# KrArunT/whisper-rust-ort

Hardware: AMD Instinct MI355X
Metric: rtfx: audio seconds transcribed per wall second (whisper-base, 30 s clips, greedy 128 new tokens) (higher is better)
Workload: dtype bf16

## Files before the change

whisper-rust-ort_amd/binding.py:

```python
from __future__ import annotations

import ctypes as C
import os
from dataclasses import dataclass
from typing import List, Optional, Sequence, Tuple

import numpy as np

HERE = os.path.dirname(os.path.abspath(__file__))
LIB_PATH = os.path.join(HERE, "libwhisper_hip.so")

WH_PREC_F32, WH_PREC_BF16, WH_PREC_FP8, WH_PREC_F16X3 = 0, 1, 2, 3
PRECISIONS = {"f32": WH_PREC_F32, "bf16": WH_PREC_BF16, "fp8": WH_PREC_FP8, "f16x3": WH_PREC_F16X3}
WH_N_FRAMES, WH_CLIP_SAMPLES = 3000, 480000
WH_PCM_S16, WH_PCM_U8, WH_PCM_F32 = 0, 1, 2
WH_MAX_CHANNELS = 64
PCM_FORMATS = {np.dtype(np.int16): WH_PCM_S16, np.dtype(np.uint8): WH_PCM_U8, np.dtype(np.float32): WH_PCM_F32}
KG_NAMES = ("mel", "enc_gemm", "enc_attn", "dec_cross_attn", "dec_gemm", "dec_other")

STATUS = {0: "WH_OK", 1: "WH_ERR_EMPTY_AUDIO", 2: "WH_ERR_BAD_SHAPE", 3: "WH_ERR_STATE", 4: "WH_ERR_ARG",
          5: "WH_ERR_NOMEM", 6: "WH_ERR_HIP", 7: "WH_ERR_IO", 8: "WH_ERR_UNSUPPORTED"}

EXPORTS = ("wh_model_load", "wh_model_create", "wh_model_free", "wh_model_get_dims", "wh_model_precision",
           "wh_model_export_tensor", "wh_ctx_create", "wh_ctx_create_ex", "wh_ctx_free", "wh_ctx_cross_mode", "wh_ctx_placement", "wh_last_error", "wh_get_timings",
# ... 325 lines not shown
            rc = self.lib.wh_ctx_create_ex(model.h, C.byref(o), C.byref(h))
        if rc:
            raise WhisperHipError(rc, (self.lib.wh_last_error(None) or b"").decode())
        self.h = h

    def _check(self, rc: int):
        if rc:
            raise WhisperHipError(rc, (self.lib.wh_last_error(self.h) or b"").decode())

    @property
    def cross_mode(self) -> int:
        return int(self.lib.wh_ctx_cross_mode(self.h))

    @property
    def placement(self) -> dict:
        a, b = C.c_float(0), C.c_float(0)
        n = int(self.lib.wh_ctx_placement(self.h, C.byref(a), C.byref(b)))
        return {"workspaces_timed": n, "first_us_per_launch": float(a.value), "kept_us_per_launch": float(b.value)}

    def debug_set_step_split(self, rows: int):
        self._check(self.lib.wh_debug_set_step_split(self.h, C.c_int(rows)))

    @property
    def step_split(self) -> int:
        return int(self.lib.wh_debug_get_step_split(self.h))

    def debug_set_step_free(self, on: bool):
        self._check(self.lib.wh_debug_set_step_free(self.h, C.c_int(1 if on else 0)))

    @property
    def step_free(self) -> int:
        return int(self.lib.wh_debug_get_step_free(self.h))

    def set_timestamp_rules(self, tb: int, no_timestamps: int = -1, max_initial_index: int = 50):
        r = WhTimestampRules(C.sizeof(WhTimestampRules), tb, no_timestamps, max_initial_index)
        self._check(self.lib.wh_ctx_set_timestamp_rules(self.h, C.byref(r)))

    def clear_timestamp_rules(self):
        self._check(self.lib.wh_ctx_set_timestamp_rules(self.h, None))

    def set_logprobs(self, no_speech: int = -1, sot_index: int = 0):
        o = WhLogprobOpts(C.sizeof(WhLogprobOpts), no_speech, sot_index)
        self._check(self.lib.wh_ctx_set_logprobs(self.h, C.byref(o)))

    def clear_logprobs(self):
        self._check(self.lib.wh_ctx_set_logprobs(self.h, None))

    def logprobs(self) -> Tuple[List[np.ndarray], Optional[np.ndarray]]:
        n = C.c_size_t(0)
        self._check(self.lib.wh_get_logprobs(self.h, None, 0, None, 0, C.byref(n)))
        k = int(n.value)
        lens = list(self._gen_lens)
        assert len(lens) == k, (len(lens), k)
        cap = max(1, max(lens, default=0))
        lp = np.zeros((max(1, k), cap), np.float32)
        ns = np.zeros(max(1, k), np.float32)
        rc = self.lib.wh_get_logprobs(self.h, _f32(lp), cap, _f32(ns), k, C.byref(n))
        if rc == 3:
            ns = None
            rc = self.lib.wh_get_logprobs(self.h, _f32(lp), cap, None, k, C.byref(n))
        self._check(rc)
        return [lp[i, : lens[i]].copy() for i in range(k)], (ns[:k] if ns is not None else None)

    def set_language_detection(self, ids: Sequence[int], sot_index: int = 0):
        a = np.ascontiguousarray(list(ids), np.int64)
        o = WhLanguageOpts(C.sizeof(WhLanguageOpts), _i64(a) if a.size else None, a.size, sot_index)
# ... 614 lines not shown
```

whisper-rust-ort_amd/build.py:

```python
from __future__ import annotations

import os
import subprocess
import sys
from concurrent.futures import ThreadPoolExecutor

HERE = os.path.dirname(os.path.abspath(__file__))
CSRC = os.path.join(HERE, "csrc")
OUT = os.path.join(HERE, "libwhisper_hip.so")
SOURCES = ["wh_lm_head.hip", "wh_dec_gemm.hip", "wh_mel.hip", "wh_ingest.hip", "wh_gemm.hip", "wh_gemm8.hip", "wh_gemm8x.hip", "wh_gemm8_mx.hip", "wh_mlp.hip", "wh_attn.hip", "wh_dec_attn.hip", "wh_dec_tile.hip", "wh_cross_es.hip", "wh_cross_es8.hip", "wh_cross_es3.hip", "wh_fp8.hip", "wh_align.hip", "wh_beam.hip", "wh_sample.hip", "wh_score.hip", "wh_model.cpp", "wh_ctx.cpp", "wh_options.cpp", "wh_encode_host.cpp", "wh_decode_host.cpp", "wh_score_host.cpp", "wh_api.cpp"]
HEADERS = ["wh_common.h", "wh_es_common.h", "wh_dec_epilogue.h", "wh_kernels.h", "wh_lm_tile.h", "wh_internal.h", "wh_host_shared.h", "wh_step.h", "wh_ingest_desc.h", "wh_json.h", "../../include/whisper_hip.h"]
FLAGS = ["--offload-arch=gfx950", "-O3", "-fPIC", "-std=c++17", "-pthread", "-Wall", "-Wno-unused-function", "-Wno-unused-value", "-Wno-unused-result",
         "-mllvm", "-amdgpu-mfma-vgpr-form=1", "-x", "hip"]


EXTRA_FLAGS = {"wh_attn.hip": ["-fno-honor-nans"], "wh_cross_es.hip": ["-fno-honor-nans"], "wh_cross_es8.hip": ["-fno-honor-nans"], "wh_cross_es3.hip": ["-fno-honor-nans"]}


def _stale(target: str, deps) -> bool:
    if not os.path.exists(target):
        return True
    t = os.path.getmtime(target)
    return any(os.path.getmtime(d) > t for d in deps)


def build(verbose: bool = False, force: bool = False) -> str:
    hipcc = os.environ.get("HIPCC", "/opt/rocm/bin/hipcc")
    objdir = os.path.join(HERE, "build")
    os.makedirs(objdir, exist_ok=True)
    hdrs = [os.path.join(CSRC, h) for h in HEADERS]

    def compile_one(src: str) -> str:
        s = os.path.join(CSRC, src)
        o = os.path.join(objdir, src + ".o")
        if force or _stale(o, [s] + hdrs):
            cmd = [hipcc] + FLAGS + EXTRA_FLAGS.get(src, []) + ["-c", s, "-o", o]
            if verbose:
                print(" ".join(cmd), flush=True)
            subprocess.check_call(cmd)
        return o

    with ThreadPoolExecutor(max_workers=min(6, os.cpu_count() or 1)) as ex:
        objs = list(ex.map(compile_one, SOURCES))
    if force or _stale(OUT, objs):
        cmd = [hipcc, "--offload-arch=gfx950", "-shared", "-fPIC", "-pthread", "-o", OUT] + objs
        if verbose:
            print(" ".join(cmd), flush=True)
        subprocess.check_call(cmd)
    build_host(verbose, force)
    build_tools(verbose, force)
    return OUT


TOOLS = os.path.join(HERE, "..", "tools")


def build_tools(verbose: bool = False, force: bool = False) -> None:
    hipcc = os.environ.get("HIPCC", "/opt/rocm/bin/hipcc")
    for name, kernel_src in (("mx_mfma_check", "wh_gemm8_mx.hip"), ("mx_gemm_check", "wh_gemm8_mx.hip"), ("mlp_check", "wh_mlp.hip"), ("es16_check", "wh_cross_es.hip"), ("es8_check", "wh_cross_es8.hip"), ("es3_check", "wh_cross_es3.hip"), ("align_check", "wh_align.hip")):
        src, exe = os.path.join(TOOLS, name + ".hip"), os.path.join(TOOLS, name)
        deps = [src, os.path.join(CSRC, kernel_src), os.path.join(CSRC, "wh_common.h"), os.path.join(CSRC, "wh_es_common.h"), os.path.join(CSRC, "wh_dec_epilogue.h"), os.path.join(CSRC, "wh_kernels.h")]
        if force or _stale(exe, deps):
            cmd = [hipcc, "--offload-arch=gfx950", "-O3", "-std=c++17", "-mllvm", "-amdgpu-mfma-vgpr-form=1"] + EXTRA_FLAGS.get(kernel_src, []) + ["-w", "-I", CSRC, src, "-o", exe]
            if verbose:
                print(" ".join(cmd), flush=True)
            subprocess.check_call(cmd)
    for name in ("dec_gemm_check", "enc_check", "dec_attn_check", "lm_check"):
        src, exe = os.path.join(TOOLS, name + ".cpp"), os.path.join(TOOLS, name)
        if force or _stale(exe, [src, OUT, os.path.join(CSRC, "wh_kernels.h")]):
            cmd = [hipcc, "--offload-arch=gfx950", "-O2", "-std=c++17", "-w", src, "-o", exe, "-L" + HERE, "-lwhisper_hip", "-Wl,-rpath,$ORIGIN/../whisper-rust-ort_amd"]
            if verbose:
                print(" ".join(cmd), flush=True)
            subprocess.check_call(cmd)


HOST = os.path.join(HERE, "host")
HOST_SO = os.path.join(HERE, "libwh_host.so")
CLI = os.path.join(HERE, "whisper_bench")


def build_host(verbose: bool = False, force: bool = False) -> None:
    gxx = os.environ.get("CXX", "g++")
    import ctypes
    try:
        ctypes.CDLL("libz.so.1")
    except OSError as e:
        raise RuntimeError(f"libz.so.1 is missing: whisper_bench --temperature and libwh_host.so's compression_ratio need zlib ({e})") from e
    hdr =[os.path.join(HOST, "wh_host.h"), os.path.join(HOST, "wh_unicode_lower.h"), os.path.join(CSRC, "wh_json.h"), os.path.join(HERE, "..", "include", "whisper_hip.h")]
    src = os.path.join(HOST, "wh_host_capi.cpp")
    if force or _stale(HOST_SO, [src] + hdr):
        cmd = [gxx, "-O2", "-std=c++17", "-fPIC", "-shared", "-Wall", "-o", HOST_SO, src, "-ldl"]
        if verbose:
            print(" ".join(cmd), flush=True)
        subprocess.check_call(cmd)
    src = os.path.join(HOST, "whisper_bench.cpp")
    if force or _stale(CLI, [src, OUT] + hdr):
        cmd = [gxx, "-O2", "-std=c++17", "-Wall", "-pthread", "-D__HIP_PLATFORM_AMD__", "-I/opt/rocm/include", "-o", CLI, src, "-L" + HERE, "-lwhisper_hip",
               "-Wl,-rpath,$ORIGIN", "-Wl,-rpath,/opt/rocm/lib", "-L/opt/rocm/lib", "-lamdhip64", "-ldl"]
        if verbose:
            print(" ".join(cmd), flush=True)
# ... 6 lines not shown
```

whisper-rust-ort_amd/csrc/wh_ctx.cpp:

```cpp
#include "wh_host_shared.h"

using namespace wh;

namespace wh {

int fail(wh_ctx* c, int code, const char* fmt, ...) {
    char buf[1024];
    va_list ap;
    va_start(ap, fmt);
    vsnprintf(buf, sizeof buf, fmt, ap);
    va_end(ap);
    if (c) c->err = buf;
    wh_set_error("%s", buf);
    return code;
}

void prof_reset(wh_ctx* c) {
    for (int g = 0; g < WH_KG_COUNT; g++) { c->prof_used[g] = 0; c->prof_ms[g] = 0; c->prof_launches[g] = 0; }
}
void prof_collect(wh_ctx* c) {
    if (!c->prof) return;
    for (int g = 0; g < WH_KG_COUNT; g++) {
        double ms = 0;
        for (size_t i = 0; i < c->prof_used[g]; i++) {
// ... 148 lines not shown
    c->sm.timing = getenv("WH_SAMPLE_TIMING") != nullptr;
    c->sc.timing = getenv("WH_SCORE_TIMING") != nullptr;
    const wh_dims& D = m->dims;
    const size_t B = max_batch, d = D.d_model, S = D.n_audio_ctx, F = D.ffn, C = D.n_mels, esz = m->esz;
    const size_t Ld = D.dec_layers, H = D.n_heads, TC = D.n_text_ctx;
    c->ldv = (int)align_up(S, 64);
    c->tok_ld = D.n_text_ctx + 1;
    c->mpad = (int)align_up(B, B > 16 ? 64 : 16);
    c->cross_splits = (int)std::min<size_t>(32, std::max<size_t>(1, 256 / B));
    if (m->prec == WH_PREC_BF16 && d > 512 && d % 256 == 0)
        c->cross_splits = (int)std::min<size_t>(32, std::max<size_t>(1, 512 / (B * (d / 256))));
    const size_t n_tiles = (D.vocab + 15) / 16;
    Carver cv;
    const size_t o_pcm = cv.take(B * WH_CLIP_SAMPLES * 4), o_raw = cv.take(B * C * RAW_LD * 4);
    const size_t o_melstage = cv.take(C * WH_N_FRAMES * 4);
    const size_t o_melT = cv.take((B * TOK_ROWS * C + 256) * esz), o_h1 = cv.take((B * H1_ROWS * d + 256) * esz);
    const size_t o_x = cv.take(B * S * d * 4), o_xn = cv.take(B * S * d * esz), o_qk = cv.take(B * S * 2 * d * esz);
    c->enc_fold = m->prec == WH_PREC_BF16 && max_batch > WH_SMALL_CTX_CLIPS && d >= 256 && (d % 64) == 0 && (F % 64) == 0 && S >= 256 && (S % 4) == 0 &&
                  m->cross_kv_wf != nullptr && wh_gemm8_enabled() && getenv("WH_NO_ENC_FOLD") == nullptr;
    c->enc_mlp = c->enc_fold && d == 512 && F >= 128 && (F % 128) == 0 && !(getenv("WH_ENC_MLP") && atoi(getenv("WH_ENC_MLP")) == 0);
    const size_t o_vT = cv.take(B * d * c->ldv * esz), o_att = cv.take(B * S * d * esz), o_h = c->enc_mlp ? 0 : cv.take(B * S * F * esz);
    const size_t o_enc = cv.take(B * S * d * esz), o_encf = cv.take(B * S * d * 4);
    c->cross_es = m->cross_es && max_batch >= 256;
    if (opts->flags & WH_CTX_CROSS_ES_ON) c->cross_es = m->cross_es;
    if (opts->flags & WH_CTX_CROSS_ES_OFF) c->cross_es = false;
    if (const char* e = getenv("WH_CROSS_ES")) c->cross_es = m->cross_es && atoi(e) != 0;
    if ((opts->flags & WH_CTX_CROSS_ES_ON) && !m->cross_es) {
        delete c;
        wh_set_error("wh_ctx_create_ex: WH_CTX_CROSS_ES_ON needs a bf16 or f16x3 model of whisper-base geometry (d_model 512, 8 heads)");
        return WH_ERR_UNSUPPORTED;
    }
    c->dec_tile = m->prec == WH_PREC_F16X3 && max_batch >= 1024;
    if (const char* e = getenv("WH_DEC_TILE")) c->dec_tile = (m->prec == WH_PREC_BF16 || m->prec == WH_PREC_F16X3) && atoi(e) != 0;
    c->es_rows = (int)S + 20;
    if (const char* e = getenv("WH_ES_PAD")) c->es_rows = (int)S + std::max(0, atoi(e));
    c->es_rows_cap = c->es_rows;
    if (const char* e = getenv("WH_ES_PAD_MAX")) c->es_rows_cap = std::max(c->es_rows, (int)S + atoi(e));
    const size_t o_ckv = cv.take(c->cross_es ? B * (size_t)c->es_rows_cap * d * esz : Ld * 2 * B * S * d * esz);
    const bool f8 = m->prec == WH_PREC_FP8;
    const bool f8kv = f8 && !c->cross_es;
    const size_t o_ckv8 = f8kv ? cv.take(Ld * 2 * B * S * d) : 0, o_kvam = f8kv ? cv.take(Ld * 2 * B * H * 4) : 0;
    auto mx_k = [](size_t k) { return k >= 256 && (k % 128) == 0; };
    c->mx_ok = f8 && mx_k(d) && mx_k(F) && wh_mx_ln_width((int)d) && S >= 256 && (S % 4) == 0 && getenv("WH_NO_MX") == nullptr;
    const size_t o_xn8 = c->mx_ok ? cv.take(B * S * d) : 0, o_xn8s = c->mx_ok ? cv.take(B * S * 4 * wh_mx_nkp((int)d)) : 0;
    const size_t o_h8 = c->mx_ok ? cv.take(B * S * F) : 0, o_h8s = c->mx_ok ? cv.take(B * S * 4 * wh_mx_nkp((int)F)) : 0;
    const size_t o_xb = c->enc_fold ? cv.take(B * S * d * 2) : 0, o_epart = c->enc_fold ? cv.take((d / 64) * B * S * 2 * 4) : 0;
    const size_t o_estat = c->enc_fold ? cv.take(B * S * 2 * 4) : 0, o_eshift = c->enc_fold ? cv.take(B * S * 4) : 0, o_eshift0 = c->enc_fold ? cv.take(B * S * 4) : 0;
    const size_t o_sk = cv.take(Ld * B * H * TC * WH_HEAD_DIM * esz), o_sv = cv.take(Ld * B * H * TC * WH_HEAD_DIM * esz);
    const size_t MP = (size_t)c->mpad;
    const size_t o_dx = cv.take(B * d * 4), o_dxn = cv.take(MP * d * esz), o_dqkv = cv.take(B * 3 * d * esz);
    const size_t o_dxs = cv.take(MP * d * esz), o_lnp = cv.take((d / 16) * MP * 2 * 4), o_dsh = cv.take(MP * 4);
    const size_t o_datt = cv.take(MP * d * esz), o_dq = cv.take(B * d * esz), o_dh = cv.take(MP * F * esz);
    const size_t o_dqe = c->cross_es ? cv.take(B * H * d * 4) : 0, o_dctx = c->cross_es ? cv.take(MP * H * d * esz) : 0;
    const size_t o_dq32 = c->cross_es ? cv.take(B * d * 4) : 0;
    const size_t o_cpart = cv.take(B * c->cross_splits * d * 4), o_cml = cv.take(B * c->cross_splits * H * 2 * 4);
    const size_t o_pv = cv.take(MP * (n_tiles + 4) * 4), o_pi = cv.take(MP * (n_tiles + 4) * 4);
    const size_t o_feed = cv.take(B * c->tok_ld * 4), o_out = cv.take(B * c->tok_ld * 4);
    const size_t o_nout = cv.take(B * 4), o_done = cv.take(B * 4), o_forced = cv.take(TC * 4), o_pos = cv.take(2 * 4);
    const size_t o_stk = cv.take(2 * 4);
    const size_t o_m1 = cv.take((D.vocab / 32 + 1) * 4), o_m2 = cv.take((D.vocab / 32 + 1) * 4);
    const size_t o_ns = cv.take(B * 4), o_nf = cv.take(B * 4), o_si = cv.take(B * 4), o_fs = cv.take(B * 4), o_gm = cv.take(B * 4);
    const size_t o_lsel = cv.take(B * 4);
    hipError_t he = hipMalloc(&c->ws.p, cv.off);
    if (he != hipSuccess) { delete c; return wh_fail_hip(he, "hipMalloc(workspace)", __FILE__, __LINE__); }
    c->ws.bytes = cv.off;
    he = hipMemset(c->ws, 0, c->ws.bytes);
// ... 133 lines not shown
    for (auto& e : c->free_ev) hipEventDestroy(e);
    if (c->s_split) hipStreamDestroy(c->s_split);
    for (int g = 0; g < WH_KG_COUNT; g++)
        for (auto& e : c->prof_events[g]) { hipEventDestroy(e.first); hipEventDestroy(e.second); }
    for (auto& e : c->ev)
        if (e) hipEventDestroy(e);
    for (auto& set : c->enc_ev)
        for (auto& e : set)
            if (e) hipEventDestroy(e);
    if (c->ev_enc_done) hipEventDestroy(c->ev_enc_done);
    if (c->ev_kv_done) hipEventDestroy(c->ev_kv_done);
    if (c->s_enc && c->s_enc != c->stream) hipStreamDestroy(c->s_enc);
    if (c->stream) hipStreamDestroy(c->stream);
    c->reset_option_results();
    if (c->s_copy) { hipStreamSynchronize(c->s_copy); hipStreamDestroy(c->s_copy); }
    if (c->ev_h2d) hipEventDestroy(c->ev_h2d);
    delete c;
}

int wh_ctx_cross_mode(const wh_ctx* c) { return c ? (c->cross_es ? 1 : 0) : -1; }

extern "C" int wh_debug_set_es_pad(wh_ctx* c, int pad_rows) {
    if (!c || !c->cross_es || pad_rows < 0 || c->m->dims.n_audio_ctx + pad_rows > c->es_rows_cap) return WH_ERR_ARG;
    c->es_rows = c->m->dims.n_audio_ctx + pad_rows;
    c->have_enc = false;
    return WH_OK;
}

extern "C" int wh_debug_set_step_split(wh_ctx* c, int rows) {
    if (!c || rows < 0) return WH_ERR_ARG;
    c->dbg_split = rows;
    return WH_OK;
}
extern "C" int wh_debug_get_step_split(const wh_ctx* c) { return c ? c->last_split : -1; }
extern "C" int wh_debug_set_step_free(wh_ctx* c, int on) {
    if (!c) return WH_ERR_ARG;
    c->dbg_free = on != 0;
    return WH_OK;
}
extern "C" int wh_debug_get_step_free(const wh_ctx* c) { return c ? c->last_free : -1; }

const char* wh_last_error(const wh_ctx* c) { return c ? c->err.c_str() : wh_global_error().c_str(); }

int wh_get_timings(const wh_ctx* c, wh_timing* out) {
    if (!c || !out) return WH_ERR_ARG;
    *out = c->timing;
    return WH_OK;
}

int wh_profile_enable(wh_ctx* c, int group_mask) {
    if (!c) return WH_ERR_ARG;
    c->prof = (group_mask & 0xFFFF) != 0;
    c->prof_mask = group_mask & 0xFFFF;
    c->prof_stride = (group_mask >> 16) & 0xFFFF;
    return WH_OK;
}
int wh_profile_get(const wh_ctx* c, double* ms, int64_t* launches) {
    if (!c || !ms || !launches) return WH_ERR_ARG;
    for (int g = 0; g < WH_KG_COUNT; g++) { ms[g] = c->prof_ms[g]; launches[g] = c->prof_launches[g]; }
    return WH_OK;
}

}
```

whisper-rust-ort_amd/csrc/wh_decode_host.cpp:

```cpp
#include "wh_step.h"

namespace wh {

void pack_mask(const int64_t* a, size_t na, const int64_t* b, size_t nb, int vocab, std::vector<unsigned>& out) {
    out.assign((size_t)vocab / 32 + 1, 0u);
    for (size_t i = 0; i < na; i++)
        if (a[i] >= 0 && a[i] < vocab) out[a[i] >> 5] |= 1u << (a[i] & 31);
    for (size_t i = 0; i < nb; i++)
        if (b[i] >= 0 && b[i] < vocab) out[b[i] >> 5] |= 1u << (b[i] & 31);
}


struct DecodePlan {
    wh_ctx::StepKey key;
    int P = 0, NEW = 0;
    int Nmax = 0;
    std::vector<int> plen;
    std::vector<const int64_t*> pids;
    bool lang_det = false, lang_fix = false, lp_probe = false;
    int lang_slot = -1;
    int lang_pos = -1, probe_pos = -1;
    bool want_logits = false;
    size_t n_lrows = 0;
    std::vector<int> sel_map;
// ... 27 lines not shown
        for (int i = 0; i < P; i++)
            if (i != lang_slot && c->ts.no_ts >= 0 && p->prompt[i] == c->ts.no_ts) return fail(c, WH_ERR_ARG, "decode: the prompt holds <|notimestamps|> while timestamp rules are on");
    }
    pl.lp_probe = c->lp.on && c->lp.no_speech >= 0;
    if (pl.lp_probe && c->lp.sot_index >= P - 1)
        return fail(c, WH_ERR_ARG, "decode: the no-speech probe's sot_index %d is not below n_prompt - 1 (%d)", c->lp.sot_index, P - 1);
    pl.plen.assign(nb, 0);
    pl.pids.assign(nb, nullptr);
    if (c->pfx.on)
        for (int b = 0; b < nb; b++) {
            pl.pids[b] = prefix_of(c, c->pfx.win_base, b / K, &pl.plen[b]);
            pl.Nmax = std::max(pl.Nmax, pl.plen[b]);
        }
    if (pl.lang_det) pl.lang_pos = pl.Nmax + c->lang.sot_index;
    if (pl.lp_probe) pl.probe_pos = pl.Nmax + c->lp.sot_index;
    pl.want_logits = want_logits;
    pl.n_lrows = sel ? n_sel : (size_t)nb;
    if (want_logits && sel) {
        pl.sel_map.assign(nb, -1);
        for (size_t i = 0; i < n_sel; i++) {
            if (sel[i] < 0 || sel[i] >= nb || pl.sel_map[sel[i]] >= 0) return fail(c, WH_ERR_ARG, "decode: logits row %d outside the batch or listed twice", (int)sel[i]);
            pl.sel_map[sel[i]] = (int)i;
        }
    }
    wh_ctx::StepKey& key = pl.key;
    key.nb = nb; key.n_prompt = pl.Nmax + P; key.pfx = pl.Nmax > 0; key.eot = (int)p->eot; key.n_forced = (int)p->n_forced;
    key.logits_rows = (int)logits_rows;
    if (c->ts.on) { key.ts_begin = (int)c->ts.begin; key.ts_max_init = c->ts.max_init; }
    if (c->lp.on) key.lp_sum = c->lp.part_sum;
    if (c->rep.on) { key.rep = true; key.rep_p = c->rep.p; key.rep_n = c->rep.n; }
    if (c->al.on) { key.al_cap = NEW; key.al_gen = c->al.gen; }
    if (c->bm.on) { key.beam_k = c->bm.k; key.beam_c = c->bm.c; key.beam_buf = c->bm.buf; }
    if (c->sm.on && !sample_trivial(c)) key.sample_buf = c->sm.buf;
    key.split = choose_split(c, key);
    key.split_cus = key.split ? std::min(c->split_cus, c->dec_cus) : 0;
    key.free = choose_free(c, key, want_logits);
    return WH_OK;
}

static int upload_token_state(wh_ctx* c, const wh_decode_params* p, const DecodePlan& pl) {
    hipStream_t s = c->stream;
    const int nb = pl.key.nb, ld = c->tok_ld, Nmax = pl.Nmax, vocab = c->m->dims.vocab;
    std::vector<int> feed((size_t)nb * ld, 0);
    for (int b = 0; b < nb; b++) {
        for (int i = 0; i < pl.plen[b]; i++) feed[(size_t)b * ld + Nmax - pl.plen[b] + i] = (int)pl.pids[b][i];
        for (int i = 0; i < pl.P; i++) feed[(size_t)b * ld + Nmax + i] = i == pl.lang_slot ? (pl.lang_fix ? (int)c->lang.fixed : 0) : (int)p->prompt[i];
    }
    if (pl.key.pfx) {
        std::vector<int> off(nb);
        for (int b = 0; b < nb; b++) off[b] = Nmax - pl.plen[b];
        CTX_HIP(c, hipMemcpyAsync(c->pfx.off, off.data(), nb * 4, hipMemcpyHostToDevice, s));
        CTX_HIP(c, hipStreamSynchronize(s));
    }
    CTX_HIP(c, hipMemcpyAsync(c->feed, feed.data(), feed.size() * 4, hipMemcpyHostToDevice, s));
    CTX_HIP(c, hipMemcpyAsync(c->out_tokens, feed.data(), feed.size() * 4, hipMemcpyHostToDevice, s));
    std::vector<int> nout(nb, pl.key.n_prompt);
    CTX_HIP(c, hipMemcpyAsync(c->n_out, nout.data(), nb * 4, hipMemcpyHostToDevice, s));
    CTX_HIP(c, hipMemsetAsync(c->done, 0, nb * 4, s));
    std::vector<int> sm_done;
    std::vector<float> sm_t;
    std::vector<unsigned long long> sm_id;
    if (pl.key.sample_buf) {
        const bool lf = c->pfx.win_base >= 0;
        sm_done.resize(nb); sm_t.resize(nb); sm_id.resize(nb);
        for (int b = 0; b < nb; b++) {
            sm_done[b] = c->sm.active[lf ? 0 : b] ? 0 : 1;
// ... 706 lines not shown
        }
        for (size_t k = 0; k < c->bm.trace_clips.size(); k++) {
            if (c->bm.trace_clips[k] != clip) continue;
            wh_ctx::BeamTrace& tr = c->bm.traces[k];
            tr.K = K; tr.n_steps = ns;
            tr.parents.clear(); tr.tokens.clear(); tr.scores.clear(); tr.pool.clear();
            for (int g = 0; g < ns; g++) {
                for (int j = 0; j < K; j++) {
                    const size_t t = (size_t)g * ld + r0 + j;
                    tr.parents.push_back(trp[t]); tr.tokens.push_back(trt[t]); tr.scores.push_back(trs[t]);
                }
                tr.pool.push_back(trpool[(size_t)g * ld + clip]);
            }
        }
        c->bm.hyps.push_back(std::move(hyps));
    }
    c->bm.have = true;
    if (c->lp.on) { c->lp.have = true; c->lp.have_ns = pl.lp_probe; }
    if (logits_out)
        if (int rc = copy_kept_logits(c, pl, logits_out, sel, [&](int r) { return (size_t)nsteps[r / K]; })) return rc;
    c->timing.d2h_s = now_s() - t0;
    return WH_OK;
}

int run_decode(wh_ctx* c, int nb, const wh_decode_params* p, int64_t* tokens_out, size_t tok_stride, size_t* n_tokens_out, float* logits_out,
               size_t logits_rows, const std::function<int()>& after_kv, const int32_t* sel, size_t n_sel) {
    hipStream_t s = c->stream;
    c->cur = s;
    DecodePlan pl;
    int rc = plan_decode(c, nb, p, logits_out != nullptr, logits_rows, sel, n_sel, pl);
    if (rc) return rc;
    const wh_ctx::StepKey& key = pl.key;
    c->last_split = c->last_free = 0;
    if (key.split && (rc = ensure_split_stream(c))) return rc;
    if (c->s_enc != s) CTX_HIP(c, hipStreamWaitEvent(s, c->ev_enc_done, 0));
    CTX_HIP(c, hipEventRecord(c->ev[5], s));
    if ((rc = upload_token_state(c, p, pl)) || (rc = prepare_logits(c, pl)) || (rc = prepare_alignment(c, pl)) || (rc = project_cross_kv(c, nb, after_kv))) return rc;
    const int PP = key.n_prompt, total_pos = PP + pl.NEW - 1;
    for (int step = 0; step < std::min(PP, total_pos); step++) {
        PromptStep ps;
        ps.emits = step >= PP - 1;
        ps.lang = step == pl.lang_pos; ps.lang_col = pl.Nmax + pl.lang_slot;
        ps.probe = step == pl.probe_pos;
        launch_step(c, key, &ps);
    }
    if ((rc = run_token_loop(c, key, total_pos - PP, p->n_forced == 0)) || (rc = run_alignment(c, pl))) return rc;
    CTX_HIP(c, hipEventRecord(c->ev[3], s));
    if (key.beam_k) return read_back_beam(c, pl, tokens_out, tok_stride, n_tokens_out, logits_out, sel);
    return read_back(c, pl, tokens_out, tok_stride, n_tokens_out, logits_out, sel);
}

}
```

whisper-rust-ort_amd/csrc/wh_internal.h:

```cpp
#pragma once
#include <hip/hip_runtime.h>

#include <array>
#include <map>
#include <string>
#include <tuple>
#include <vector>

#include "../../include/whisper_hip.h"
#include "wh_kernels.h"

struct EncLayerDev {
    void *qk_w, *v_w, *o_w, *fc1_w, *fc2_w;
    float *qk_b, *v_b, *o_b, *fc1_b, *fc2_b;
    float *ln1_w, *ln1_b, *ln2_w, *ln2_b;
    float *qk_sc = nullptr, *v_sc = nullptr, *o_sc = nullptr, *fc1_sc = nullptr, *fc2_sc = nullptr;
    void *qk_w8 = nullptr, *v_w8 = nullptr, *fc1_w8 = nullptr, *fc2_w8 = nullptr;
    void *qk_wf = nullptr, *v_wf = nullptr, *fc1_wf = nullptr;
    float *qk_s = nullptr, *qk_c = nullptr, *v_s = nullptr, *v_c = nullptr, *fc1_s = nullptr, *fc1_c = nullptr;
};
struct DecLayerDev {
    void *qkv_w, *o_w, *cq_w, *co_w, *fc1_w, *fc2_w;
    float *qkv_b, *o_b, *cq_b, *co_b, *fc1_b, *fc2_b;
    float *ln1_w, *ln1_b, *ln2_w, *ln2_b, *ln3_w, *ln3_b;
// ... 150 lines not shown
    int *feed = nullptr, *out_tokens = nullptr, *n_out = nullptr, *done = nullptr, *forced = nullptr, *pos = nullptr;
    int* step_ticket = nullptr;
    unsigned *mask_first = nullptr, *mask_base = nullptr;
    DevBuf<float> logits;
    int* logits_sel = nullptr;
    DevBuf<float> pcm2;
    hipStream_t s_copy = nullptr;
    hipEvent_t ev_h2d = nullptr;
    int h2d_buf = 0;
    const float* h2d_src = nullptr;
    int h2d_n = 0;
    bool h2d_valid = false;
    std::vector<int> h2d_ns, h2d_nf;
    DevBuf<> ing_raw[2];
    DevBuf<WhIngestDesc> ing_desc;
    int ing_n = 0, ing_buf = 0;
    size_t ing_max_out = 0;
    int ing_last_n = 0, ing_last_buf = 0;
    size_t ing_last_max_out = 0;
    bool h2d_is_raw = false;
    std::vector<wh_raw_clip> h2d_raw_clips;
    struct FileSet {
        size_t n = 0;
        DevBuf<float> mel;
        DevBuf<WhFileDesc> desc;
        DevBuf<WhIngestDesc> ing;
        DevBuf<int> rows;
        std::vector<WhFileDesc> host;
    } fs;
    int tok_ld = 0;
    int mpad = 16;
    int cross_splits = 1;
    bool dec_tile = false;
    struct StepKey {
        int nb = 0, n_prompt = 0, eot = 0, n_forced = 0, logits_rows = 0;
        float* d_logits = nullptr;
        const int* d_sel = nullptr;
        int ts_begin = -1, ts_max_init = -1;
        float* lp_sum = nullptr;
        bool pfx = false;
        bool rep = false;
        float rep_p = 1.0f;
        int rep_n = 0;
        float* al_q = nullptr;
        int al_cap = 0;
        unsigned al_gen = 0;
        int beam_k = 0, beam_c = 0;
        const void* beam_buf = nullptr;
        const void* sample_buf = nullptr;
        int split = 0, split_cus = 0;
        bool free = false;
        auto members() const { return std::tie(split, split_cus, free, nb, n_prompt, eot, n_forced, logits_rows, d_logits, d_sel, ts_begin, ts_max_init, lp_sum, pfx, rep, rep_p, rep_n, al_q, al_cap, al_gen, beam_k, beam_c, beam_buf, sample_buf); }
        bool operator==(const StepKey& o) const { return members() == o.members(); }
    } step_key;
    struct TimestampRules {
        bool on = false;
        int64_t begin = 0, no_ts = -1;
        int max_init = 50;
        int ld = 0;
        DevBuf<float> logits;
        DevBuf<int> state;
        void reset_results() {}
    } ts;
    struct Logprobs {
        bool on = false;
        int64_t no_speech = -1;
        int sot_index = 0;
        DevBuf<> buf;
        float* part_sum = nullptr;
        float* tok = nullptr;
        unsigned* mask_zero = nullptr;
        float* probe_v = nullptr;
        float* ns = nullptr;
        bool have = false, have_ns = false;
        std::vector<std::vector<float>> rows;
        std::vector<float> ns_rows;
        void reset_results() { have = have_ns = false; rows.clear(); ns_rows.clear(); }
    } lp;
    struct LanguageDetection {
        bool on = false;
        int sot_index = 0;
        std::vector<int64_t> ids;
        DevBuf<> buf;
        int* d_ids = nullptr;
        float* logits = nullptr;
// ... 134 lines not shown
```

whisper-rust-ort_amd/csrc/wh_kernels.h:

```cpp
#pragma once
#include <hip/hip_runtime.h>
#include <stddef.h>
#include <vector>

#include "../../include/whisper_hip.h"

constexpr int WH_SMALL_CTX_CLIPS = 8;

struct GemmArgs {
    const void* A = nullptr;
    long lda = 0, a_bs = 0, a_zs = 0;
    const void* W = nullptr;
    long ldw = 0, w_zs = 0;
    void* C = nullptr;
    long ldc = 0, c_bs = 0, c_zs = 0;
    const float* bias = nullptr;
    int bias_mode = 0;
    const float* wscale = nullptr;
    const float* R = nullptr;
    long ldr = 0, r_bs = 0, r_zs = 0;
    int act = 0;
    int M = 0, N = 0, K = 0;
    int m_per = 1 << 30;
    int n_per = 1 << 30;
// ... 189 lines not shown
void wh_launch_lm_head_tile_x3(hipStream_t s, const SkinnyArgs& a);
int wh_lm_head_parts(int prec, const SkinnyArgs& a);
void wh_launch_argmax_finish(hipStream_t s, int prec, const float* part_val, const int* part_idx, int n_parts, int mpad, int* pos_p,
                             int* ticket, const DecodeState& st, int B, const NextEmbed& ne, const TsFinish& ts = TsFinish(),
                             const float* part_sum = nullptr,
                             const RepFinish& rep = RepFinish());
void wh_launch_nospeech_finish(hipStream_t s, const float* part_val, const float* part_sum, int n_parts, int mpad, const float* probe_v,
                               float* prob, int B, int* pos_p);
constexpr int WH_LANG_LD = 128;
struct LangHeadArgs {
    const void* X = nullptr;
    int x_mpad = 64;
    const void* W = nullptr;
    const float* bias = nullptr;
    const float* ln_s = nullptr;
    const float* ln_part = nullptr;
    int ln_tiles = 0;
    const int* ids = nullptr;
    int n_lang = 0;
    int M = 0, K = 0;
    float* out = nullptr;
};
void wh_launch_lang_head(hipStream_t s, int prec, const LangHeadArgs& a);
void wh_launch_lang_finish(hipStream_t s, const float* logits, const int* ids, int n_lang, int src_row, float* probs, int* chosen, int* feed,
                           int* out_tokens, int tok_ld, int tok_pos, int B, int* pos_p);
void wh_launch_dec_self_attn(hipStream_t s, int prec, const void* qkv, void* kc, void* vc, void* out, const int* pos_p,
                             int d, int n_heads, int tc, int B, int mpad, const int* off = nullptr);
void wh_launch_dec_cross_attn(hipStream_t s, int prec, const void* q, const void* ck, const void* cv, float* part,
                              float* ml, int S, int d, int n_heads, int splits, int B, void* out, int mpad, bool stream_nt,
                              int rows_per_clip = 1);

bool wh_cross_es_geometry(int d, int n_heads, int S);
void wh_launch_dec_qexpand(hipStream_t s, int prec, const float* q, const void* wkT, float* qe, int M, int d, int n_heads);
void wh_launch_dec_cross_attn_es(hipStream_t s, int prec, const float* qe, const void* E, void* out, int S, int e_rows, int B, int mpad, bool stream_nt, int n_cus,
                                 int rows_per_clip = 1);
void wh_launch_layernorm_es2(hipStream_t s, const float* x, const float* w, const float* b, void* y, long rows, int in_blk, int out_blk);
bool wh_es3_enabled();
void wh_launch_dec_cross_attn_es3(hipStream_t s, const float* qe, const void* E, void* out, int S, int e_rows, int B, int mpad, bool stream_nt, int n_cus);
void wh_launch_layernorm_es3(hipStream_t s, const float* x, const float* w, const float* b, void* y, long rows, int in_blk, int out_blk);
void wh_launch_dec_cross_attn_es8(hipStream_t s, const float* qe, const void* E, void* out, int S, int e_rows, int B, int mpad, bool stream_nt, int n_cus);
void wh_launch_layernorm_es8(hipStream_t s, const float* x, const float* gamma, const float* beta, void* out, long rows, int S, int e_rows);

size_t wh_cross_lds_reserve(long total_wgs, size_t own_bytes);

void wh_launch_kv_quant(hipStream_t s, const void* kv_bf16, unsigned* amax, void* kv8, long planes_x_clips, int S, int d,
                        int n_heads);
void wh_launch_dec_cross_attn8(hipStream_t s, const void* q, const void* ck, const void* cv, const float* amax_k,
                               const float* amax_v, float* part, float* ml, int S, int d, int n_heads, int splits, int B, void* out,
                               int mpad, bool stream_nt);

struct AlignLayerHeads {
    int n = 0;
    unsigned char slot[WH_MAX_ALIGN_HEADS] = {0}, head[WH_MAX_ALIGN_HEADS] = {0};
};
void wh_launch_align_copy(hipStream_t s, bool src_bf16, const void* src, long row_pitch, long head_pitch, int dk, const AlignLayerHeads& hs, const int* pos_p,
                          int first_emit, int cap, int nb, float* dst);
constexpr int WH_ALIGN_KV_F32 = 0, WH_ALIGN_KV_BF16 = 1, WH_ALIGN_ES_BF16 = 2;
struct AlignArgs {
    const float* q = nullptr;
    const void* k_base[WH_MAX_ALIGN_HEADS] = {nullptr};
    long k_clip_pitch = 0, k_row_pitch = 0;
    int dk = 0;
    const int* n_out = nullptr;
    int n_prompt = 0, cap = 0;
    const int* sb = nullptr;
    int nb = 0, n_heads = 0, S = 0, Sp = 0, clip0 = 0;
// ... 69 lines not shown
```

whisper-rust-ort_amd/csrc/wh_score_host.cpp:

```cpp
#include "wh_step.h"

namespace wh {

struct ScorePlan {
    int ncl = 0, H = 0, n_hyp = 0, P = 0, Lmax = 0, T = 0, clips_per_pass = 0;
    std::vector<int> len;
};

static int plan_score(wh_ctx* c, const wh_decode_params* p, const wh_score_input* in, float* logprob_out, size_t cap_tokens, const int32_t* logit_hyps,
                      size_t n_logit_hyps, float* logits_out, size_t cap_logits_rows, ScorePlan& pl) {
    const wh_dims& D = c->m->dims;
    if (!in || in->struct_size != sizeof(wh_score_input))
        return fail(c, WH_ERR_ARG, "wh_score_tokens: struct_size %zu, expected %zu", in ? in->struct_size : (size_t)0, sizeof(wh_score_input));
    if (!c->have_enc) return fail(c, WH_ERR_STATE, "Missing cached decoder input: encoder states (call wh_transcribe_batch or wh_encode first)");
    if (c->pre_valid) return fail(c, WH_ERR_STATE, "the resident encoder states belong to a prefetched batch that has not been transcribed yet");
    if (c->m->prec != WH_PREC_F32 && c->m->prec != WH_PREC_BF16)
        return fail(c, WH_ERR_UNSUPPORTED, "wh_score_tokens: not supported in the %s mode (only the f32 and bf16 cross-attention kernels share a clip between rows)",
                    c->m->prec == WH_PREC_FP8 ? "fp8" : "f16x3");
    const char* opt = c->ts.on ? "timestamp rules" : c->rep.on ? "repetition controls" : c->sm.on ? "sampling" : c->bm.on ? "beam search" : c->al.on ? "alignment"
                      : c->lang.on ? "language detection" : nullptr;
    if (c->pfx.on && !c->pfx.ids.empty()) opt = "a non-empty prefix";
    if (opt) return fail(c, WH_ERR_UNSUPPORTED, "wh_score_tokens: %s set on the ctx is not supported (clear it first)", opt);
    if (p->n_forced != 0) return fail(c, WH_ERR_ARG, "wh_score_tokens: forced tokens are not taken (the hypotheses are the history)");
    const int P = pl.P = (int)p->n_prompt;
// ... 109 lines not shown
    CTX_HIP(c, hipStreamSynchronize(s));
    CTX_HIP(c, hipGetLastError());
    for (int g = 0; g < G; g++)
        for (int i = 0; i < pl.len[g0 + g]; i++) {
            logprob_out[(size_t)(g0 + g) * cap_tokens + i] = lp[(size_t)g * Lmax + i];
            if (argmax_out) argmax_out[(size_t)(g0 + g) * cap_tokens + i] = am[(size_t)g * Lmax + i];
        }
    return WH_OK;
}

int run_score(wh_ctx* c, const wh_decode_params* p, const wh_score_input* in, float* logprob_out, int64_t* argmax_out, size_t cap_tokens,
              const int32_t* logit_hyps, size_t n_logit_hyps, float* logits_out, size_t cap_logits_rows) {
    ScorePlan pl;
    if (int rc = plan_score(c, p, in, logprob_out, cap_tokens, logit_hyps, n_logit_hyps, logits_out, cap_logits_rows, pl)) return rc;
    CTX_HIP(c, hipSetDevice(c->m->device));
    hipStream_t s = c->stream;
    c->cur = s;
    const wh_dims& D = c->m->dims;
    if (int rc = ensure_score_buffers(c)) return rc;
    for (size_t i = 0; i < (size_t)pl.n_hyp * cap_tokens; i++) logprob_out[i] = 0.0f;
    if (argmax_out) for (size_t i = 0; i < (size_t)pl.n_hyp * cap_tokens; i++) argmax_out[i] = 0;
    if (c->s_enc != s) CTX_HIP(c, hipStreamWaitEvent(s, c->ev_enc_done, 0));
    CTX_HIP(c, hipEventRecord(c->ev[5], s));
    std::vector<unsigned> mfirst, mbase;
    pack_mask(p->suppress, p->n_suppress, p->begin_suppress, p->n_begin_suppress, D.vocab, mfirst);
    pack_mask(p->suppress, p->n_suppress, nullptr, 0, D.vocab, mbase);
    CTX_HIP(c, hipMemcpyAsync(c->mask_first, mfirst.data(), mfirst.size() * 4, hipMemcpyHostToDevice, s));
    CTX_HIP(c, hipMemcpyAsync(c->mask_base, mbase.data(), mbase.size() * 4, hipMemcpyHostToDevice, s));
    const int pos = pl.T - 1;
    CTX_HIP(c, hipMemcpyAsync(c->pos, &pos, 4, hipMemcpyHostToDevice, s));
    CTX_HIP(c, hipStreamSynchronize(s));
    if (int rc = project_cross_kv(c, pl.ncl, nullptr)) return rc;
    wh_ctx::StepKey key;
    key.n_prompt = 1; key.eot = (int)p->eot;
    for (int clip0 = 0; clip0 < pl.ncl; clip0 += pl.clips_per_pass)
        if (int rc = score_pass(c, p, in, pl, key, clip0, std::min(pl.clips_per_pass, pl.ncl - clip0), logprob_out, argmax_out, cap_tokens, logit_hyps, n_logit_hyps,
                                logits_out, cap_logits_rows))
            return rc;
    CTX_HIP(c, hipEventRecord(c->ev[3], s));
    CTX_HIP(c, hipStreamSynchronize(s));
    c->sc.collect_timing();
    return WH_OK;
}

}

extern "C" int wh_debug_score_times(const wh_ctx* c, double* ms2) {
    if (!c || !ms2 || !c->sc.timing) return WH_ERR_ARG;
    ms2[0] = c->sc.ms[0]; ms2[1] = c->sc.ms[1];
    return WH_OK;
}
```

whisper-rust-ort_amd/csrc/wh_step.h:

```cpp
#pragma once
#include "wh_host_shared.h"

namespace wh {

void pack_mask(const int64_t* a, size_t na, const int64_t* b, size_t nb, int vocab, std::vector<unsigned>& out);
int project_cross_kv(wh_ctx* c, int nb, const std::function<int()>& after_kv);

struct StepBase {
    wh_ctx* c;
    const wh_ctx::StepKey& k;
    wh_model* m = c->m;
    const wh_dims& D = m->dims;
    hipStream_t s = c->stream;
    const int prec = m->prec, nb = k.nb, mpad = c->mpad, ln_tiles_d = D.d_model / 16;
    const long d = D.d_model, S = D.n_audio_ctx;
    const bool f8 = prec == WH_PREC_FP8, rules = k.ts_begin >= 0;
    const int rpc, ncl, clip0;
    const bool kv_nt = (c->cross_es ? 1.0 : (double)D.dec_layers * 2.0) * ncl * S * d * (f8 ? 1 : (double)m->esz) > 128.0 * 1024 * 1024;
    int row0 = 0, nr = nb, es_cus = c->dec_cus;
    int *pos = c->pos, *ticket = c->step_ticket;
    template <typename T> T* rm(T* p, long ld) const { return p + (long)row0 * ld; }
    void* rm(void* p, long ld, size_t esz) const { return (char*)p + (long)row0 * ld * (long)esz; }
    void* slab(void* p) const { return (char*)p + (long)row0 * 32 * (long)m->esz; }
    hipEvent_t q_rec = nullptr;
// ... 28 lines not shown
        a.X = slab(c->dxs); a.x_mpad = mpad;
        a.pos_p = pos; a.n_prompt = k.n_prompt;
        a.part_val = c->part_val + row0; a.part_idx = c->part_idx + row0;
        return a;
    }
    SkinnyArgs lm_head_masked(float* scratch = nullptr) const {
        SkinnyArgs a = lm_head_common();
        a.mask_first = c->mask_first; a.mask_base = c->mask_base;
        if (scratch) { a.logits = scratch; a.logits_rows = 1; a.logits_cur = true; }
        return a;
    }

    template <typename SelfAttn>
    void layer_with(int l, bool advance, SelfAttn&& self_attn) const {
        layer_head(l, self_attn);
        layer_tail(l, advance);
    }
    template <typename SelfAttn>
    void layer_head(int l, SelfAttn&& self_attn) const {
        const DecLayerDev& L = m->dec[l];
        {
            Prof pr(c, WH_KG_DEC_GEMM);
            gemm(false, ln_consumer(L.qkv_w, L.qkv_b, L.qkv_sc, L.qkv_s, 3 * d, rm(c->dqkv, 3 * d, prec == WH_PREC_F16X3 ? 4 : m->esz), (l == 0) ? 1 : ln_tiles_d));
        }
        {
            Prof pr(c, WH_KG_DEC_OTHER);
            self_attn();
        }
        {
            Prof pr(c, WH_KG_DEC_GEMM);
            gemm(true, residual_producer(L.o_w, L.o_b, L.o_sc, slab(c->datt), d, L.ln2_w));
        }
        if (c->cross_es) {
            {
                Prof pr(c, WH_KG_DEC_GEMM);
                gemm(true, ln_consumer(L.cq_w, L.cq_b, L.cq_sc, L.cq_s, d, rm(c->dq32, d), ln_tiles_d));
                wh_launch_dec_qexpand(s, prec, rm(c->dq32, d), L.cqx_w, rm(c->dqe, D.n_heads * d), nr, (int)d, D.n_heads);
            }
        } else {
            Prof pr(c, WH_KG_DEC_GEMM);
            gemm(false, ln_consumer(L.cq_w, L.cq_b, L.cq_sc, L.cq_s, d, rm(c->dq, d, prec == WH_PREC_F16X3 ? 4 : m->esz), ln_tiles_d));
        }
        after_query(l);
    }
    void layer_tail(int l, bool advance) const {
        const DecLayerDev& L = m->dec[l];
        const long kv_stride = (long)ncl * S * d;
        const long kv_clip0 = (long)(clip0 + row0) * S * d;
        if (c->cross_es) {
            if (k.al_q && c->al.layer[l].n) {
                Prof pr(c, WH_KG_DEC_OTHER);
                wh_launch_align_copy(s, false, c->dqe, (long)D.n_heads * d, d, (int)d, c->al.layer[l], c->pos, k.n_prompt - 1, k.al_cap, nb, k.al_q);
            }
            {
                Prof pr(c, WH_KG_DEC_CROSS_ATTN);
                wh_launch_dec_cross_attn_es(s, prec, rm(c->dqe, D.n_heads * d), (const char*)c->es_E + (long)(clip0 + row0) * c->es_rows * d * m->esz, slab(c->dctx), (int)S,
                                            c->es_rows, nr, mpad, kv_nt, es_cus, rpc);
            }
            {
                Prof pr(c, WH_KG_DEC_GEMM);
                SkinnyArgs a;
                a.X = slab(c->dctx); a.x_mpad = mpad; a.W = L.cv_w; a.bias = L.cv_b; a.C = slab(c->datt); a.c_mpad = mpad;
                a.M = nr; a.m_sel = nb; a.N = WH_HEAD_DIM; a.K = (int)d;
                a.zn = D.n_heads; a.x_zs = (long)(d / 32) * mpad * 32; a.w_zs = (long)WH_HEAD_DIM * d; a.c_zs = (long)(WH_HEAD_DIM / 32) * mpad * 32;
                a.bias_zs = WH_HEAD_DIM;
                if (f8) wh_launch_dec_gemm(s, WH_PREC_BF16, false, a);
                else gemm(false, a);
// ... 41 lines not shown
```

Baseline: 80910.

## Fuse decoder cross-attention Q projection with Q expansion into one kernel

Adds a new kernel that computes the LayerNorm-folded cross-attention Q projection per head and immediately expands it through the cross-key weight (split hi/lo bf16 MFMA), writing qe directly. This replaces a skinny GEMM that wrote dq32 and a separate qexpand launch, removing one launch and the intermediate round trip per decoder layer per step. It is enabled by default for bf16 with cross_es, no dec_tile, d=512 and 8 heads. The fused kernel reloads Q weights per head block and uses a hi/lo split for precision, which may cost extra MFMA work.

```diff
diff --git a/whisper-rust-ort_amd/binding.py b/whisper-rust-ort_amd/binding.py
--- a/whisper-rust-ort_amd/binding.py
+++ b/whisper-rust-ort_amd/binding.py
@@ -381,6 +381,13 @@
     def step_free(self) -> int:
         return int(self.lib.wh_debug_get_step_free(self.h))
 
+    def debug_set_dec_fuse(self, level: int):
+        self._check(self.lib.wh_debug_set_dec_fuse(self.h, C.c_int(level)))
+
+    @property
+    def dec_fuse(self) -> int:
+        return int(self.lib.wh_debug_get_dec_fuse(self.h))
+
     def set_timestamp_rules(self, tb: int, no_timestamps: int = -1, max_initial_index: int = 50):
         r = WhTimestampRules(C.sizeof(WhTimestampRules), tb, no_timestamps, max_initial_index)
         self._check(self.lib.wh_ctx_set_timestamp_rules(self.h, C.byref(r)))
diff --git a/whisper-rust-ort_amd/build.py b/whisper-rust-ort_amd/build.py
--- a/whisper-rust-ort_amd/build.py
+++ b/whisper-rust-ort_amd/build.py
@@ -8,7 +8,7 @@
 HERE = os.path.dirname(os.path.abspath(__file__))
 CSRC = os.path.join(HERE, "csrc")
 OUT = os.path.join(HERE, "libwhisper_hip.so")
-SOURCES = ["wh_lm_head.hip", "wh_dec_gemm.hip", "wh_mel.hip", "wh_ingest.hip", "wh_gemm.hip", "wh_gemm8.hip", "wh_gemm8x.hip", "wh_gemm8_mx.hip", "wh_mlp.hip", "wh_attn.hip", "wh_dec_attn.hip", "wh_dec_tile.hip", "wh_cross_es.hip", "wh_cross_es8.hip", "wh_cross_es3.hip", "wh_fp8.hip", "wh_align.hip", "wh_beam.hip", "wh_sample.hip", "wh_score.hip", "wh_model.cpp", "wh_ctx.cpp", "wh_options.cpp", "wh_encode_host.cpp", "wh_decode_host.cpp", "wh_score_host.cpp", "wh_api.cpp"]
+SOURCES = ["wh_lm_head.hip", "wh_dec_gemm.hip", "wh_mel.hip", "wh_ingest.hip", "wh_gemm.hip", "wh_gemm8.hip", "wh_gemm8x.hip", "wh_gemm8_mx.hip", "wh_mlp.hip", "wh_attn.hip", "wh_dec_attn.hip", "wh_dec_tile.hip", "wh_dec_fuse.hip", "wh_cross_es.hip", "wh_cross_es8.hip", "wh_cross_es3.hip", "wh_fp8.hip", "wh_align.hip", "wh_beam.hip", "wh_sample.hip", "wh_score.hip", "wh_model.cpp", "wh_ctx.cpp", "wh_options.cpp", "wh_encode_host.cpp", "wh_decode_host.cpp", "wh_score_host.cpp", "wh_api.cpp"]
 HEADERS = ["wh_common.h", "wh_es_common.h", "wh_dec_epilogue.h", "wh_kernels.h", "wh_lm_tile.h", "wh_internal.h", "wh_host_shared.h", "wh_step.h", "wh_ingest_desc.h", "wh_json.h", "../../include/whisper_hip.h"]
 FLAGS = ["--offload-arch=gfx950", "-O3", "-fPIC", "-std=c++17", "-pthread", "-Wall", "-Wno-unused-function", "-Wno-unused-value", "-Wno-unused-result",
          "-mllvm", "-amdgpu-mfma-vgpr-form=1", "-x", "hip"]
@@ -65,7 +65,7 @@
             if verbose:
                 print(" ".join(cmd), flush=True)
             subprocess.check_call(cmd)
-    for name in ("dec_gemm_check", "enc_check", "dec_attn_check", "lm_check"):
+    for name in ("dec_gemm_check", "enc_check", "dec_attn_check", "lm_check", "dec_fuse_check"):
         src, exe = os.path.join(TOOLS, name + ".cpp"), os.path.join(TOOLS, name)
         if force or _stale(exe, [src, OUT, os.path.join(CSRC, "wh_kernels.h")]):
             cmd = [hipcc, "--offload-arch=gfx950", "-O2", "-std=c++17", "-w", src, "-o", exe, "-L" + HERE, "-lwhisper_hip", "-Wl,-rpath,$ORIGIN/../whisper-rust-ort_amd"]
diff --git a/whisper-rust-ort_amd/csrc/wh_ctx.cpp b/whisper-rust-ort_amd/csrc/wh_ctx.cpp
--- a/whisper-rust-ort_amd/csrc/wh_ctx.cpp
+++ b/whisper-rust-ort_amd/csrc/wh_ctx.cpp
@@ -204,6 +204,9 @@
     }
     c->dec_tile = m->prec == WH_PREC_F16X3 && max_batch >= 1024;
     if (const char* e = getenv("WH_DEC_TILE")) c->dec_tile = (m->prec == WH_PREC_BF16 || m->prec == WH_PREC_F16X3) && atoi(e) != 0;
+    c->dec_fuse_max = (c->cross_es && !c->dec_tile && wh_dec_fuse_geometry(m->prec, (int)d, (int)H)) ? 1 : 0;
+    c->dec_fuse = c->dec_fuse_max;
+    if (const char* e = getenv("WH_DEC_FUSE")) c->dec_fuse = std::min(c->dec_fuse_max, std::max(0, atoi(e)));
     c->es_rows = (int)S + 20;
     if (const char* e = getenv("WH_ES_PAD")) c->es_rows = (int)S + std::max(0, atoi(e));
     c->es_rows_cap = c->es_rows;
@@ -403,6 +406,13 @@
     c->dbg_split = rows;
     return WH_OK;
 }
+extern "C" int wh_debug_set_dec_fuse(wh_ctx* c, int level) {
+    if (!c || level < 0 || level > 2) return WH_ERR_ARG;
+    drop_step_graph(c);
+    c->dec_fuse = std::min(level, c->dec_fuse_max);
+    return WH_OK;
+}
+extern "C" int wh_debug_get_dec_fuse(const wh_ctx* c) { return c ? c->last_fuse : -1; }
 extern "C" int wh_debug_get_step_split(const wh_ctx* c) { return c ? c->last_split : -1; }
 extern "C" int wh_debug_set_step_free(wh_ctx* c, int on) {
     if (!c) return WH_ERR_ARG;
diff --git a/whisper-rust-ort_amd/csrc/wh_dec_fuse.hip b/whisper-rust-ort_amd/csrc/wh_dec_fuse.hip
--- /dev/null
+++ b/whisper-rust-ort_amd/csrc/wh_dec_fuse.hip
@@ -0,0 +1,131 @@
+#include "wh_common.h"
+#include "wh_dec_epilogue.h"
+#include "wh_kernels.h"
+
+int wh_dbg_fuse_rows = 0;
+
+namespace {
+
+constexpr int FD = 512, FH = 8;
+template <int FROWS>
+struct FuseLds {
+    static constexpr size_t LNQ = (size_t)4 * (FROWS / 4) * 64 * 16, QHI = LNQ + 4 * FROWS * 8, QLO = QHI + 2 * FROWS * 32 * 2, BYTES = QLO + 2 * FROWS * 32 * 2;
+};
+
+template <int MT>
+__global__ __launch_bounds__(256) void k_dec_fuse_q(DecFuseQArgs a) {
+    constexpr int FROWS = 16 * MT, TILES = 4 * MT;
+    typedef FuseLds<FROWS> L;
+    extern __shared__ __attribute__((aligned(128))) char smem[];
+    f32x4* red = reinterpret_cast<f32x4*>(smem);
+    float* lnq = reinterpret_cast<float*>(smem + L::LNQ);
+    bf16* qhi = reinterpret_cast<bf16*>(smem + L::QHI);
+    bf16* qlo = reinterpret_cast<bf16*>(smem + L::QLO);
+    const int tid = threadIdx.x, lane = tid & 63, wave = tid >> 6, fl = lane & 15, fg = lane >> 4;
+    const int h = blockIdx.y, m0 = blockIdx.x * FROWS;
+    const int kb = wave * (FD / 4);
+    bf16x8 wq[4][4], xq[4][MT];
+#pragma unroll
+    for (int nt = 0; nt < 4; nt++)
+#pragma unroll
+        for (int i = 0; i < 4; i++) wq[nt][i] = load_frag<bf16>((const bf16*)a.cq_w + (long)(h * WH_HEAD_DIM + nt * 16 + fl) * FD + kb + 32 * i + 8 * fg);
+#pragma unroll
+    for (int t = 0; t < MT; t++) {
+        const int m = min(m0 + 16 * t + fl, a.M - 1);
+#pragma unroll
+        for (int i = 0; i < 4; i++) xq[i][t] = load_frag<bf16>((const bf16*)a.xs + ((long)(kb / 32 + i) * a.mpad + m) * 32 + 8 * fg);
+    }
+    bf16x8 wf[8][2];
+#pragma unroll
+    for (int nt = 0; nt < 8; nt++)
+#pragma unroll
+        for (int ks = 0; ks < 2; ks++)
+            wf[nt][ks] = load_frag<bf16>((const bf16*)a.cqx_w + ((long)h * FD + (8 * wave + nt) * 16 + fl) * WH_HEAD_DIM + 32 * ks + 8 * fg);
+    if (tid < 4 * FROWS) {
+        const int r = tid % FROWS, q = tid / FROWS;
+        float s1, s2;
+        ln_partial_sum(a.lnpart, FD / 16, a.mpad, min(m0 + r, a.M - 1), q, 4, s1, s2);
+        ln_part_store<FROWS>(lnq, r, q, s1, s2);
+    }
+    f32x4 acc[4][MT];
+#pragma unroll
+    for (int nt = 0; nt < 4; nt++)
+#pragma unroll
+        for (int t = 0; t < MT; t++) acc[nt][t] = f32x4{0, 0, 0, 0};
+#pragma unroll
+    for (int i = 0; i < 4; i++)
+#pragma unroll
+        for (int nt = 0; nt < 4; nt++)
+#pragma unroll
+            for (int t = 0; t < MT; t++) mma16(acc[nt][t], wq[nt][i], xq[i][t]);
+#pragma unroll
+    for (int nt = 0; nt < 4; nt++)
+#pragma unroll
+        for (int t = 0; t < MT; t++) red[(wave * TILES + nt * MT + t) * 64 + lane] = acc[nt][t];
+    __syncthreads();
+    {
+        const int nt = wave, en = nt * 16 + 4 * fg;
+        const f32x4 b = *reinterpret_cast<const f32x4*>(a.cq_b + h * WH_HEAD_DIM + en), sv = *reinterpret_cast<const f32x4*>(a.cq_s + h * WH_HEAD_DIM + en);
+#pragma unroll
+        for (int t = 0; t < MT; t++) {
+            const int tile = nt * MT + t, row = 16 * t + fl;
+            f32x4 s = red[(0 * TILES + tile) * 64 + lane];
+#pragma unroll
+            for (int w = 1; w < 4; w++) {
+                const f32x4 o = red[(w * TILES + tile) * 64 + lane];
+                s[0] += o[0]; s[1] += o[1]; s[2] += o[2]; s[3] += o[3];
+            }
+            float mean, rstd;
+            ln_row_stats<FROWS>(lnq, row, FD, mean, rstd);
+            float hi[4], lo[4];
+#pragma unroll
+            for (int e = 0; e < 4; e++) {
+                float v = wh_ln_fold(wh_scale(s[e], 1.0f), mean, rstd, sv[e], b[e]);
+                v += 0.0f;
+                const bf16 hb = (bf16)v;
+                hi[e] = (float)hb;
+                lo[e] = v - (float)hb;
+            }
+            store4(qhi + slab_idx(row, en, FROWS), hi[0], hi[1], hi[2], hi[3]);
+            store4(qlo + slab_idx(row, en, FROWS), lo[0], lo[1], lo[2], lo[3]);
+            if (h == 0 && nt == 0 && fg == 0 && m0 + row < a.M) a.shift[m0 + row] += mean;
+        }
+    }
+    __syncthreads();
+    bf16x8 xh[2][MT], xl[2][MT];
+#pragma unroll
+    for (int ks = 0; ks < 2; ks++)
+#pragma unroll
+        for (int t = 0; t < MT; t++) {
+            xh[ks][t] = load_frag<bf16>(qhi + (ks * FROWS + 16 * t + fl) * 32 + 8 * fg);
+            xl[ks][t] = load_frag<bf16>(qlo + (ks * FROWS + 16 * t + fl) * 32 + 8 * fg);
+        }
+#pragma unroll
+    for (int t = 0; t < MT; t++) {
+        const int m = m0 + 16 * t + fl;
+#pragma unroll
+        for (int nt = 0; nt < 8; nt++) {
+            f32x4 o = {0, 0, 0, 0};
+#pragma unroll
+            for (int ks = 0; ks < 2; ks++) {
+                o = __builtin_amdgcn_mfma_f32_16x16x32_bf16(wf[nt][ks], xl[ks][t], o, 0, 0, 0);
+                o = __builtin_amdgcn_mfma_f32_16x16x32_bf16(wf[nt][ks], xh[ks][t], o, 0, 0, 0);
+            }
+            if (m < a.M) *reinterpret_cast<f32x4*>(a.qe + ((long)m * FH + h) * FD + (8 * wave + nt) * 16 + 4 * fg) = o;
+        }
+    }
+}
+
+}
+
+bool wh_dec_fuse_geometry(int prec, int d, int n_heads) { return prec == WH_PREC_BF16 && d == FD && n_heads == FH; }
+
+void wh_launch_dec_fuse_q(hipStream_t s, const DecFuseQArgs& a) {
+    if (a.M <= 0) return;
+    if ((wh_dbg_fuse_rows ? wh_dbg_fuse_rows : a.M > 1024 ? 64 : 32) == 64) {
+        set_max_smem(k_dec_fuse_q<4>, FuseLds<64>::BYTES);
+        hipLaunchKernelGGL(k_dec_fuse_q<4>, dim3((a.M + 63) / 64, FH), dim3(256), FuseLds<64>::BYTES, s, a);
+    } else {
+        hipLaunchKernelGGL(k_dec_fuse_q<2>, dim3((a.M + 31) / 32, FH), dim3(256), FuseLds<32>::BYTES, s, a);
+    }
+}
diff --git a/whisper-rust-ort_amd/csrc/wh_decode_host.cpp b/whisper-rust-ort_amd/csrc/wh_decode_host.cpp
--- a/whisper-rust-ort_amd/csrc/wh_decode_host.cpp
+++ b/whisper-rust-ort_amd/csrc/wh_decode_host.cpp
@@ -83,6 +83,7 @@
     if (c->al.on) { key.al_cap = NEW; key.al_gen = c->al.gen; }
     if (c->bm.on) { key.beam_k = c->bm.k; key.beam_c = c->bm.c; key.beam_buf = c->bm.buf; }
     if (c->sm.on && !sample_trivial(c)) key.sample_buf = c->sm.buf;
+    key.fuse = c->dec_fuse;
     key.split = choose_split(c, key);
     key.split_cus = key.split ? std::min(c->split_cus, c->dec_cus) : 0;
     key.free = choose_free(c, key, want_logits);
@@ -855,6 +856,7 @@
     if (rc) return rc;
     const wh_ctx::StepKey& key = pl.key;
     c->last_split = c->last_free = 0;
+    c->last_fuse = key.fuse;
     if (key.split && (rc = ensure_split_stream(c))) return rc;
     if (c->s_enc != s) CTX_HIP(c, hipStreamWaitEvent(s, c->ev_enc_done, 0));
     CTX_HIP(c, hipEventRecord(c->ev[5], s));
diff --git a/whisper-rust-ort_amd/csrc/wh_internal.h b/whisper-rust-ort_amd/csrc/wh_internal.h
--- a/whisper-rust-ort_amd/csrc/wh_internal.h
+++ b/whisper-rust-ort_amd/csrc/wh_internal.h
@@ -206,6 +206,7 @@
     int mpad = 16;
     int cross_splits = 1;
     bool dec_tile = false;
+    int dec_fuse_max = 0, dec_fuse = 0, last_fuse = 0;
     struct StepKey {
         int nb = 0, n_prompt = 0, eot = 0, n_forced = 0, logits_rows = 0;
         float* d_logits = nullptr;
@@ -224,7 +225,8 @@
         const void* sample_buf = nullptr;
         int split = 0, split_cus = 0;
         bool free = false;
-        auto members() const { return std::tie(split, split_cus, free, nb, n_prompt, eot, n_forced, logits_rows, d_logits, d_sel, ts_begin, ts_max_init, lp_sum, pfx, rep, rep_p, rep_n, al_q, al_cap, al_gen, beam_k, beam_c, beam_buf, sample_buf); }
+        int fuse = 0;
+        auto members() const { return std::tie(fuse, split, split_cus, free, nb, n_prompt, eot, n_forced, logits_rows, d_logits, d_sel, ts_begin, ts_max_init, lp_sum, pfx, rep, rep_p, rep_n, al_q, al_cap, al_gen, beam_k, beam_c, beam_buf, sample_buf); }
         bool operator==(const StepKey& o) const { return members() == o.members(); }
     } step_key;
     struct TimestampRules {
diff --git a/whisper-rust-ort_amd/csrc/wh_kernels.h b/whisper-rust-ort_amd/csrc/wh_kernels.h
--- a/whisper-rust-ort_amd/csrc/wh_kernels.h
+++ b/whisper-rust-ort_amd/csrc/wh_kernels.h
@@ -245,6 +245,19 @@
 
 bool wh_cross_es_geometry(int d, int n_heads, int S);
 void wh_launch_dec_qexpand(hipStream_t s, int prec, const float* q, const void* wkT, float* qe, int M, int d, int n_heads);
+bool wh_dec_fuse_geometry(int prec, int d, int n_heads);
+struct DecFuseQArgs {
+    const void* xs = nullptr;
+    const float* lnpart = nullptr;
+    float* shift = nullptr;
+    const void* cq_w = nullptr;
+    const float* cq_b = nullptr;
+    const float* cq_s = nullptr;
+    const void* cqx_w = nullptr;
+    float* qe = nullptr;
+    int M = 0, mpad = 0;
+};
+void wh_launch_dec_fuse_q(hipStream_t s, const DecFuseQArgs& a);
 void wh_launch_dec_cross_attn_es(hipStream_t s, int prec, const float* qe, const void* E, void* out, int S, int e_rows, int B, int mpad, bool stream_nt, int n_cus,
                                  int rows_per_clip = 1);
 void wh_launch_layernorm_es2(hipStream_t s, const float* x, const float* w, const float* b, void* y, long rows, int in_blk, int out_blk);
diff --git a/whisper-rust-ort_amd/csrc/wh_score_host.cpp b/whisper-rust-ort_amd/csrc/wh_score_host.cpp
--- a/whisper-rust-ort_amd/csrc/wh_score_host.cpp
+++ b/whisper-rust-ort_amd/csrc/wh_score_host.cpp
@@ -165,7 +165,7 @@
     CTX_HIP(c, hipStreamSynchronize(s));
     if (int rc = project_cross_kv(c, pl.ncl, nullptr)) return rc;
     wh_ctx::StepKey key;
-    key.n_prompt = 1; key.eot = (int)p->eot;
+    key.n_prompt = 1; key.eot = (int)p->eot; key.fuse = c->last_fuse = c->dec_fuse;
     for (int clip0 = 0; clip0 < pl.ncl; clip0 += pl.clips_per_pass)
         if (int rc = score_pass(c, p, in, pl, key, clip0, std::min(pl.clips_per_pass, pl.ncl - clip0), logprob_out, argmax_out, cap_tokens, logit_hyps, n_logit_hyps,
                                 logits_out, cap_logits_rows))
diff --git a/whisper-rust-ort_amd/csrc/wh_step.h b/whisper-rust-ort_amd/csrc/wh_step.h
--- a/whisper-rust-ort_amd/csrc/wh_step.h
+++ b/whisper-rust-ort_amd/csrc/wh_step.h
@@ -84,7 +84,13 @@
             gemm(true, residual_producer(L.o_w, L.o_b, L.o_sc, slab(c->datt), d, L.ln2_w));
         }
         if (c->cross_es) {
-            {
+            if (k.fuse) {
+                Prof pr(c, WH_KG_DEC_GEMM);
+                DecFuseQArgs a;
+                a.xs = slab(c->dxs); a.lnpart = rm(c->lnpart, 2); a.shift = rm(c->dshift, 1); a.cq_w = L.cq_w; a.cq_b = L.cq_b; a.cq_s = L.cq_s; a.cqx_w = L.cqx_w;
+                a.qe = rm(c->dqe, D.n_heads * d); a.M = nr; a.mpad = mpad;
+                wh_launch_dec_fuse_q(s, a);
+            } else {
                 Prof pr(c, WH_KG_DEC_GEMM);
                 gemm(true, ln_consumer(L.cq_w, L.cq_b, L.cq_sc, L.cq_s, d, rm(c->dq32, d), ln_tiles_d));
                 wh_launch_dec_qexpand(s, prec, rm(c->dq32, d), L.cqx_w, rm(c->dqe, D.n_heads * d), nr, (int)d, D.n_heads);
```

After: 81620, median of 6. Within noise of the previous version (+0.9%).
